# tohtsky/irspack

Measured on AMD Instinct MI355X. Metric: iALS user+item updates/sec at k=64, ML-20M-shape CSR, higher is better.
Workload: dtype f32; 1 GPU; ml20m-shape synthetic CSR 138493x26744 nnz=20004796, iALS k=64 fp32, solver=CHOLESKY; loss=IALSPP, balance=equal

## Files before the change

irspack_amd/csrc/ials.hip:

```cpp
#include <algorithm>
#include <chrono>
#include <cmath>
#include <cstdlib>
#include <atomic>
#include <cstring>
#include <map>
#include <memory>
#include <numeric>
#include <random>
#include <sstream>
#include <future>
#include <thread>

#include "common.hpp"
#include "comm.hpp"
#include "host_prep.hpp"

#include <hip/hip_ext.h>
#include "ials_kernels.hpp"
#include "ials_chol16.hpp"
#include "ials_wg_kernels.hpp"
#include "ials_wg16_kernels.hpp"
#include "ials_pp_kernels.hpp"
#include "ials_feature_kernels.hpp"
#include "ials_ridge_kernels.hpp"
#include "ials_short_kernels.hpp"
#include "ials_gk_kernels.hpp"
#include "ials_eig_kernels.hpp"
#include "ials_mf_kernels.hpp"

namespace irs {

std::string &last_error() {
  static thread_local std::string e;
  return e;
}

void require_device(int device) {
  int n = 0;
  hipError_t e = hipGetDeviceCount(&n);
  if (e != hipSuccess || n <= 0)
    throw std::runtime_error(
        "irspack_amd: no HIP device is visible; the gfx950 kernels cannot run "
        "(there is no CPU fallback).");
  if (device < 0 || device >= n)
    throw std::invalid_argument("irspack_amd: device index out of range.");
  IRS_HIP(hipSetDevice(device));
}

namespace ials {

static int padded_k(int64_t K) {
  if (K <= 16) return 16;
  if (K <= 32) return 32;
  if (K <= 64) return 64;
  return static_cast<int>(ceil_div(K, 64) * 64);
}

static int chunk_size() {
  static int v = [] {
    const char *e = std::getenv("IRSPACK_AMD_IALS_CHUNK");
    int c = e ? std::atoi(e) : 1024;
    if (c < 64) c = 64;
    return (c + 3) & ~3;
  }();
  return v;
}

static int max_chunks() { return 256; }

struct Side {
  int64_t n_rows = 0, n_other = 0, row_begin = 0, row_end = 0, nnz = 0;
  DeviceBuffer<int32_t> indptr, indices;
  DeviceBuffer<float> data, reg;
  DeviceBuffer<Task> tasks;
  DeviceBuffer<SplitRow> split;
  DeviceBuffer<FoldGroup> fold;
  int32_t n_fold = 0;
  DeviceBuffer<int32_t> rows_by_len;
  int32_t n_tasks = 0, n_split = 0, n_slots = 0, n_long = 0;
  int32_t n_short = 0, n_short16 = 0, n_short8 = 0;
  int64_t long_entries = 0;
  DeviceBuffer<MfLongRow> mf_lrows;
  DeviceBuffer<MfChunk> mf_chunks;
  int32_t mf_n_lrows = 0, mf_n_chunks = 0, mf_class[MF_CLASSES + 1] = {};
  bool unit = false;
  bool positive = false;
  float reg_min = 0.f;
  bool has_empty = false;
  bool entries_ready = false, indptr_ready = false;

  void alloc_entries(size_t ne, hipStream_t s) {
    indices.alloc(ne + 320);
    data.alloc(ne + 320);
    IRS_HIP(hipMemsetAsync(indices.ptr + ne, 0, 320 * sizeof(int32_t), s));
    IRS_HIP(hipMemsetAsync(data.ptr + ne, 0, 320 * sizeof(float), s));
    entries_ready = true;
  }
  void upload_entries(const HostCsr &m, hipStream_t s) {
    const size_t ne = static_cast<size_t>(m.indptr[m.rows]);
    alloc_entries(ne, s);
    if (ne) {
      IRS_HIP(hipMemcpyAsync(indices.ptr, m.idx(), ne * sizeof(int32_t), hipMemcpyHostToDevice, s));
      if (m.data.size() == ne) {
        IRS_HIP(hipMemcpyAsync(data.ptr, m.data.data(), ne * sizeof(float), hipMemcpyHostToDevice, s));
      } else {
        check_arg(m.flags_known && m.unit, "internal: a value array is missing.");
        IRS_HIP(hipMemsetD32Async(reinterpret_cast<hipDeviceptr_t>(data.ptr), 0x3f800000, ne, s));
      }
    }
    IRS_HIP(hipStreamSynchronize(s));
  }
  void upload_indptr(const HostCsr &m, hipStream_t s) {
    std::vector<int32_t> ip32(m.rows + 1);
    for (int64_t r = 0; r <= m.rows; r++) ip32[r] = static_cast<int32_t>(m.indptr[r]);
    indptr.upload(ip32, s);
    IRS_HIP(hipStreamSynchronize(s));
    indptr_ready = true;
  }

  void build(const HostCsr &m, int64_t rb, int64_t re, const irs_ials_model_config &cfg,
             hipStream_t s, const Side *share = nullptr) {
    n_rows = m.rows;
    n_other = m.cols;
    row_begin = rb;
    row_end = re;
    nnz = m.indptr[m.rows];
    if (share) {
      unit = share->unit;
// ... 79 lines not shown
      data.borrow(share->data);
    } else {
      if (!indptr_ready) indptr.upload(ip32, s);
      if (!entries_ready) upload_entries(m, s);
    }
    {
      std::vector<int32_t> order(re - rb);
      {
        int32_t max_len = 0;
        for (int64_t r = rb; r < re; r++) max_len = std::max(max_len, ip32[r + 1] - ip32[r]);
        std::vector<int32_t> start(static_cast<size_t>(max_len) + 2, 0);
        for (int64_t r = rb; r < re; r++) start[max_len - (ip32[r + 1] - ip32[r]) + 1]++;
        for (size_t i = 1; i < start.size(); i++) start[i] += start[i - 1];
        for (int64_t r = rb; r < re; r++)
          order[start[max_len - (ip32[r + 1] - ip32[r])]++] = static_cast<int32_t>(r);
      }
      rows_by_len.upload(order, s);
      if (cfg.K > 128 && cfg.K <= 256) {
        size_t i = 0;
        for (int c = 0; c < MF_CLASSES; c++) {
          mf_class[c] = static_cast<int32_t>(i);
          const int32_t lower = c + 1 < MF_CLASSES ? MF_CAPS[c + 1] : -1;
          while (i < order.size() && ip32[order[i] + 1] - ip32[order[i]] > lower) i++;
        }
        mf_class[MF_CLASSES] = static_cast<int32_t>(order.size());
        std::vector<MfLongRow> lr;
        std::vector<MfChunk> ch;
        for (int32_t k = 0; k < mf_class[1]; k++) {
          const int32_t r = order[k], b = ip32[r], e = ip32[r + 1], nz = e - b;
          const int32_t nch = (nz + MF_CHUNK - 1) / MF_CHUNK;
          const int32_t per = (((nz + nch - 1) / nch) + 15) & ~15;
          MfLongRow L{r, static_cast<int32_t>(ch.size()), 0, 0};
          for (int32_t c = b; c < e; c += per) {
            ch.push_back(MfChunk{k, c, std::min(c + per, e), 0});
            L.n_chunks++;
          }
          lr.push_back(L);
        }
        mf_n_lrows = static_cast<int32_t>(lr.size());
        mf_n_chunks = static_cast<int32_t>(ch.size());
        mf_lrows.upload(lr, s);
        mf_chunks.upload(ch, s);
        IRS_HIP(hipStreamSynchronize(s));
      }
      n_long = 0;
      while (n_long < static_cast<int32_t>(order.size()) &&
             ip32[order[n_long] + 1] - ip32[order[n_long]] > 2048)
        n_long++;
    }
    if (share) reg.borrow(share->reg);
    else reg.upload(regs, s);
    tasks.upload(tk, s);
    split.upload(sp, s);
    n_fold = static_cast<int32_t>(fg.size());
    fold.upload(fg, s);
    IRS_HIP(hipStreamSynchronize(s));
  }
};

struct Profiler {
  struct Rec {
    const char *name;
    hipEvent_t a, b;
  };
  bool enabled = false;
  bool dominant_only = false;
  const char *dominant_suffix = "_user";
  bool skip(const char *name) const {
    if (!enabled) return true;
    if (!dominant_only) return false;
    const size_t n = std::strlen(name), m = std::strlen(dominant_suffix);
    return std::strncmp(name, "ials_solve_", 11) != 0 || n < m || std::strcmp(name + n - m, dominant_suffix) != 0;
  }
  bool region_open = false;
  std::vector<Rec> recs;
  std::map<std::string, std::pair<double, int64_t>> totals;
  void begin(const char *name, hipStream_t s) {
    region_open = !skip(name);
    if (!region_open) return;
    Rec r{name, nullptr, nullptr};
    IRS_HIP(hipEventCreate(&r.a));
    IRS_HIP(hipEventCreate(&r.b));
    IRS_HIP(hipEventRecord(r.a, s));
    recs.push_back(r);
  }
  void end(hipStream_t s) {
    if (!region_open) return;
    region_open = false;
    IRS_HIP(hipEventRecord(recs.back().b, s));
  }
  template <class... Args, class F = void (*)(Args...)>
  void launch(const char *name, F kernel, dim3 grid, dim3 block, size_t lds, hipStream_t s, Args... args) {
    if (skip(name)) {
      hipLaunchKernelGGL(kernel, grid, block, lds, s, args...);
      return;
    }
    Rec r{name, nullptr, nullptr};
    IRS_HIP(hipEventCreate(&r.a));
    IRS_HIP(hipEventCreate(&r.b));
    if (dominant_only) {
      IRS_HIP(hipEventRecord(r.a, s));
      hipLaunchKernelGGL(kernel, grid, block, lds, s, args...);
      IRS_HIP(hipEventRecord(r.b, s));
    } else {
      hipExtLaunchKernelGGL(kernel, grid, block, static_cast<uint32_t>(lds), s, r.a, r.b, 0, args...);
    }
// ... 29 lines not shown
  int64_t K = 0, n_users = 0, n_items = 0;
  int KP = 0, T = 0;
  int device = 0;
  hipStream_t stream = nullptr;
  hipStream_t stream2 = nullptr;
  hipEvent_t ev_fork = nullptr, ev_join = nullptr;
  hipStream_t stream3 = nullptr;
  hipEvent_t ev_fork3 = nullptr, ev_join3 = nullptr;
  bool has_X = false;
  bool whole = true;
  irs_ials_shard shard{0, 0, 0, 0};
  DeviceBuffer<float> factor[2];
  Side side[2];
  DeviceBuffer<float> P_raw[2], P[2], P_acc[2], P_accL[2];
  DeviceBuffer<float> gram_partial, split_partial, row_loss;
  DeviceBuffer<double> loss_sum;
  DeviceBuffer<int32_t> err_flag;
  DeviceBuffer<float> prior[2];
  bool has_prior[2] = {false, false};
  int64_t n_feat[2] = {0, 0};
  DeviceBuffer<int32_t> f_indptr[2], f_indices[2], ft_indptr[2], ft_indices[2];
  DeviceBuffer<float> f_data[2], ft_data[2], f_W[2], f_rhs[2], f_part[2];
  int f_chunks[2] = {1, 1};
  int64_t w_rows[2] = {0, 0};
  DeviceBuffer<float> f_L[2], f_sol[2], f_gpart;
  bool ridge_ready[2] = {false, false};
  int64_t epoch = 0;
  DeviceBuffer<float> pp_pred;
  DeviceBuffer<int32_t> pp_llt_sink;
  DeviceBuffer<float> pp_pblk;
  DeviceBuffer<float> pp_px;
  DeviceBuffer<float> gk_sys, gk_delta;
  DeviceBuffer<float> eig_Qrows, eig_Qcols, eig_lam, eig_stats, eig_table, eig_xt, eig_xt2;
  DeviceBuffer<double> eig_Qd[2];
  bool eig_warm[2] = {false, false};
  int *eig_resident = nullptr;
  int eig_token = 0;
  float eig_stats_host[4] = {0, 0, 0, 0};
  bool opt_eig = true;
  DeviceBuffer<float> mf_vec, mf_xs, mf_rs, mf_partial, mf_r2;
  DeviceBuffer<int32_t> mf_done;
  bool opt_mf = true;
  bool gram_prefetched[2] = {false, false};
  std::vector<std::unique_ptr<Side>> chunk_side[2];
  int32_t eig_last = 0;
  bool gk() const { return KP > 256; }
  Profiler prof;
  bool opt_wave128 = true, opt_unit = true, opt_short = true, opt_wg16 = true;
  bool opt_short2 = true;
  bool opt_pp_direct = true;
  bool opt_pp_chain = true;
  bool opt_pp_fork = true;
  bool opt_bf16x3 = false;

  int64_t rows_of(int which) const { return which == 0 ? n_users : n_items; }
};

namespace {

#define IRS_DISPATCH_T(t, ...)                                                      \
  switch (t) {                                                                      \
    case 1: { constexpr int TT = 1; __VA_ARGS__; } break;                           \
    case 2: { constexpr int TT = 2; __VA_ARGS__; } break;                           \
    case 4: { constexpr int TT = 4; __VA_ARGS__; } break;                           \
    default:                                                                        \
      throw std::invalid_argument("irspack_amd: unsupported padded latent dimension."); \
  }
#define IRS_DISPATCH_T8(t, ...)                                                     \
  switch (t) {                                                                      \
    case 1: { constexpr int TT = 1; __VA_ARGS__; } break;                           \
    case 2: { constexpr int TT = 2; __VA_ARGS__; } break;                           \
    case 4: { constexpr int TT = 4; __VA_ARGS__; } break;                           \
    case 8: { constexpr int TT = 8; __VA_ARGS__; } break;                           \
    default:                                                                        \
      throw std::invalid_argument("irspack_amd: unsupported padded latent dimension."); \
  }
#define IRS_DISPATCH_TW(t, ...)                                                     \
  switch (t) {                                                                      \
    case 8: { constexpr int TT = 8; __VA_ARGS__; } break;                           \
    case 12: { constexpr int TT = 12; __VA_ARGS__; } break;                         \
    case 16: { constexpr int TT = 16; __VA_ARGS__; } break;                         \
    default:                                                                        \
      throw std::invalid_argument("irspack_amd: unsupported padded latent dimension."); \
  }
#define IRS_DISPATCH_ANY(t, ...)                                                    \
  switch (t) {                                                                      \
    case 1: { constexpr int TT = 1; __VA_ARGS__; } break;                           \
    case 2: { constexpr int TT = 2; __VA_ARGS__; } break;                           \
    case 4: { constexpr int TT = 4; __VA_ARGS__; } break;                           \
    case 8: { constexpr int TT = 8; __VA_ARGS__; } break;                           \
    case 12: { constexpr int TT = 12; __VA_ARGS__; } break;                         \
    case 16: { constexpr int TT = 16; __VA_ARGS__; } break;                         \
    default:                                                                        \
      throw std::invalid_argument("irspack_amd: unsupported padded latent dimension."); \
  }

void validate_config(const irs_ials_model_config &c) {
  check_arg(c.K >= 1, "K must be positive.");
  check_arg(c.K <= 32768, "irspack_amd: n_components above 32768 is not supported.");
  check_arg(c.loss_type == IRS_LOSS_ORIGINAL || c.loss_type == IRS_LOSS_IALSPP,
            "unknown loss_type.");
}

void read_switches(irs_ials_trainer *t);

void alloc_common(irs_ials_trainer *t) {
// ... 344 lines not shown
        PpParams ps = p;
        ps.rows = p.rows + n_long;
        ps.n_rows = n_rows - n_long;
        hipLaunchKernelGGL(kernel, dim3(ceil_div(ps.n_rows, 4)), dim3(256), lds, s2, ps);
      }
      if (fork) {
        IRS_HIP(hipEventRecord(t->ev_join, s2));
        IRS_HIP(hipStreamWaitEvent(t->stream, t->ev_join, 0));
      }
      t->prof.end(t->stream);
    }
  };
  const bool single = p.sub >= p.K;
  const bool chained = !single && TS == 4 && aligned && p.chain && p.sub == 64 && p.K > 64;
#define IRS_PP_LAUNCH(TSV, AL)                                                                        \
  do {                                                                                                \
    if (single)                                                                                       \
      launch(ialspp_long_kernel<TSV, AL, 1>, PpLongGeo<TSV>::LDS_FLOATS, ialspp_kernel<TSV, AL, 1>,   \
             PpGeo<TSV>::LDS_FLOATS);                                                                 \
    else                                                                                              \
      launch(ialspp_long_kernel<TSV, AL, 0>, PpLongGeo<TSV>::LDS_FLOATS, ialspp_kernel<TSV, AL, 0>,   \
             PpGeo<TSV>::LDS_FLOATS);                                                                 \
  } while (0)
  switch (TS * 2 + (aligned ? 1 : 0)) {
    case 2:
    case 3: IRS_PP_LAUNCH(1, true); break;
    case 4: IRS_PP_LAUNCH(2, false); break;
    case 5: IRS_PP_LAUNCH(2, true); break;
    case 8: IRS_PP_LAUNCH(4, false); break;
    default:
      if (chained)
        launch(ialspp_long_kernel<4, true, 2>, PpLongGeo<4>::LDS_FLOATS, ialspp_kernel<4, true, 2>,
               PpGeo<4>::LDS_FLOATS);
      else
        IRS_PP_LAUNCH(4, true);
      break;
  }
#undef IRS_PP_LAUNCH
  IRS_HIP(hipGetLastError());
}

void read_switches(irs_ials_trainer *t) {
  t->opt_wave128 = env_flag("IRSPACK_AMD_IALS_WAVE128", true);
  t->opt_unit = env_flag("IRSPACK_AMD_IALS_UNIT", true);
  t->opt_short = env_flag("IRSPACK_AMD_IALS_SHORT", true);
  t->opt_short2 = env_flag("IRSPACK_AMD_IALS_SHORT2", true);
  t->opt_pp_direct = env_flag("IRSPACK_AMD_IALSPP_DIRECT", true);
  t->opt_pp_chain = env_flag("IRSPACK_AMD_IALSPP_CHAIN", true);
  t->opt_pp_fork = env_flag("IRSPACK_AMD_IALSPP_FORK", true);
  t->opt_wg16 = env_flag("IRSPACK_AMD_IALS_WG16", true);
  t->opt_bf16x3 = env_flag("IRSPACK_AMD_IALS_BF16X3", true);
  t->opt_eig = env_flag("IRSPACK_AMD_IALS_EIG", true);
  t->opt_mf = env_flag("IRSPACK_AMD_IALS_MF", true);
}

void launch_eigen(irs_ials_trainer *t, int pidx, hipStream_t stream) {
  const int KP = t->KP;
  t->eig_Qrows.alloc(static_cast<size_t>(KP) * KP);
  t->eig_Qcols.alloc(static_cast<size_t>(KP) * KP);
  t->eig_lam.alloc(KP);
  t->eig_stats.alloc(4);
  t->eig_Qd[pidx].alloc(static_cast<size_t>(KP) * KP);
  if (!t->eig_resident) {
    IRS_HIP(hipHostMalloc(reinterpret_cast<void **>(&t->eig_resident), sizeof(int), hipHostMallocCoherent));
    *t->eig_resident = 0;
  }
  EigOut o{t->eig_Qrows.ptr, t->eig_Qcols.ptr, t->eig_lam.ptr, t->eig_stats.ptr, t->eig_Qd[pidx].ptr,
           t->eig_resident, ++t->eig_token};
  const int warm = t->eig_warm[pidx] ? 1 : 0;
  t->eig_warm[pidx] = true;
  const size_t lds = static_cast<size_t>(KP) * KP * sizeof(double);
  auto launch = [&](auto kernel) {
    IRS_HIP(hipFuncSetAttribute(reinterpret_cast<const void *>(kernel),
                                hipFuncAttributeMaxDynamicSharedMemorySize, static_cast<int>(lds)));
    t->prof.begin("eig_jacobi", stream);
    hipLaunchKernelGGL(kernel, dim3(1), dim3(1024), lds, stream,
                       static_cast<const float *>(t->P[pidx].ptr), static_cast<int>(t->K), o, warm);
    t->prof.end(stream);
  };
  if (KP == 128) launch(eig_jacobi_kernel<128>);
  else launch(eig_jacobi_kernel<64>);
  IRS_HIP(hipGetLastError());
}

bool eig_begin(irs_ials_trainer *t, Side &sd, int pidx, bool cg) {
  t->eig_last = 0;
  const int KP = t->KP;
  if (!t->opt_eig || (KP != 64 && KP != 128) || !sd.positive || sd.n_short <= 0) return false;
  if (static_cast<double>(sd.n_short) * KP * KP * KP < 3e11) return false;
  const double ratio = cg ? 64.0 : 8.0;
  if (static_cast<double>(sd.n_short) * KP < ratio * static_cast<double>(sd.n_other)) return false;
  if (!t->stream2) {
    IRS_HIP(hipStreamCreateWithFlags(&t->stream2, hipStreamNonBlocking));
    IRS_HIP(hipEventCreateWithFlags(&t->ev_fork, hipEventDisableTiming));
    IRS_HIP(hipEventCreateWithFlags(&t->ev_join, hipEventDisableTiming));
  }
  IRS_HIP(hipEventRecord(t->ev_fork, t->stream));
  IRS_HIP(hipStreamWaitEvent(t->stream2, t->ev_fork, 0));
  launch_eigen(t, pidx, t->stream2);
  const auto t0 = std::chrono::steady_clock::now();
  bool seen = false;
  int spins = 0;
  while (!(seen = __atomic_load_n(t->eig_resident, __ATOMIC_ACQUIRE) == t->eig_token) &&
         std::chrono::steady_clock::now() - t0 < std::chrono::milliseconds(200))
    if (++spins > 2000) std::this_thread::yield();
  if (!seen) {
// ... 334 lines not shown
    const int n_regular = sd.n_tasks - sd.n_short;
    int n_cu = 0;
    IRS_HIP(hipDeviceGetAttribute(&n_cu, hipDeviceAttributeMultiprocessorCount, t->device));
    t->prof.begin(pidx == 0 ? "ials_short_cg_user" : "ials_short_cg_item", short_stream);
    IRS_DISPATCH_T8(t->T, {
      constexpr int KPP = 16 * TT;
      const size_t lds = ShortGeo<KPP>::LDS_BYTES;
      auto launch = [&](auto kernel, int first, int count, int nr) {
        if (count <= 0) return;
        IRS_HIP(hipFuncSetAttribute(reinterpret_cast<const void *>(kernel),
                                    hipFuncAttributeMaxDynamicSharedMemorySize,
                                    static_cast<int>(lds)));
        const int grid = static_cast<int>(
            std::min<int64_t>(ceil_div(count, SHORT_WAVES * nr), 2 * std::max(n_cu, 1)));
        hipLaunchKernelGGL(kernel, dim3(grid), dim3(64 * SHORT_WAVES), lds, short_stream, p,
                           t->P[pidx].ptr, first, count);
      };
      if (t->opt_short2) {
        launch(ials_cg_short_kernel<KPP, 32, 1>, n_regular, sd.n_short - sd.n_short16, 1);
        launch(ials_cg_short_kernel<KPP, 16, 2>, sd.n_tasks - sd.n_short16, sd.n_short16, 2);
      } else {
        launch(ials_cg_short_kernel<KPP, 32, 1>, n_regular, sd.n_short - sd.n_short16, 1);
        launch(ials_cg_short_kernel<KPP, 16, 1>, sd.n_tasks - sd.n_short16, sd.n_short16, 1);
      }
    });
    t->prof.end(short_stream);
  };
  const bool eig_cand = prior == nullptr && !pp_direct && other == t->factor[1 - pidx].ptr &&
                        eig_begin(t, sd, pidx, cg);
  bool short_forked = false;
  if (eig_cand) {
    n_regular = sd.n_tasks - sd.n_short;
  } else if (short_cg_ok) {
    if (sd.n_short >= 65536) {
      if (!t->stream2) {
        IRS_HIP(hipStreamCreateWithFlags(&t->stream2, hipStreamNonBlocking));
        IRS_HIP(hipEventCreateWithFlags(&t->ev_fork, hipEventDisableTiming));
        IRS_HIP(hipEventCreateWithFlags(&t->ev_join, hipEventDisableTiming));
      }
      IRS_HIP(hipEventRecord(t->ev_fork, t->stream));
      IRS_HIP(hipStreamWaitEvent(t->stream2, t->ev_fork, 0));
      short_stream = t->stream2;
      short_forked = true;
    }
    launch_short_cg();
    short_stream = t->stream;
    n_regular = sd.n_tasks - sd.n_short;
  }
  auto fold_partials = [&](int partial_floats) {
    if (sd.n_fold <= 0) return;
    t->prof.launch("ials_fold_partials", fold_partials_kernel, dim3(sd.n_fold, ceil_div(partial_floats / 4, 256)),
                   dim3(256), 0, t->stream, t->split_partial.ptr, partial_floats, sd.fold.ptr);
  };
  auto launch_dense = [&](const Task *tasks_begin, int count, bool with_split) {
  const int n_regular = count;
  p.tasks = tasks_begin;
  p.n_tasks = count;
  if (!cg && (t->T >= 12 || (t->T == 8 && !t->opt_wave128)) && t->opt_wg16) {
    IRS_DISPATCH_TW(t->T, {
      using G = Geo<TT>;
      constexpr size_t lds = WgChol<TT>::LDS_FLOATS * sizeof(float);
      t->split_partial.alloc(static_cast<size_t>(std::max(sd.n_slots, 1)) * G::PARTIAL_FLOATS);
      p.partials = t->split_partial.ptr;
      auto launch = [&](auto kernel, int n_items, const char *name) {
        if (n_items <= 0) return;
        IRS_HIP(hipFuncSetAttribute(reinterpret_cast<const void *>(kernel),
                                    hipFuncAttributeMaxDynamicSharedMemorySize,
                                    static_cast<int>(lds)));
        t->prof.begin(name, t->stream);
        hipLaunchKernelGGL(kernel, dim3(n_items), dim3(256), lds, t->stream, p);
        t->prof.end(t->stream);
      };
      launch(ials_wg16_cholesky_kernel<TT, 0>, n_regular, kNames[0][0][pidx]);
      if (with_split) fold_partials(G::PARTIAL_FLOATS);
      if (with_split) launch(ials_wg16_cholesky_kernel<TT, 1>, sd.n_split, kNames[0][1][pidx]);
    });
  } else if (t->T == 8 && t->opt_wave128) {
    using G = Geo<8>;
    t->split_partial.alloc(static_cast<size_t>(std::max(sd.n_slots, 1)) * G::PARTIAL_FLOATS);
    p.partials = t->split_partial.ptr;
    if (n_regular > 0) {
      t->prof.begin(kNames[cg][0][pidx], t->stream);
      const bool x3_any = sd.unit && t->opt_unit && other == t->factor[1 - pidx].ptr && t->opt_bf16x3;
      const bool x3 = x3_any && (cg || sd.long_entries >= int64_t(320) * std::max(n_regular, 1));
      if (cg && x3)
        hipLaunchKernelGGL((ials_solve_kernel<8, 1, 0, true, true>), dim3(n_regular), dim3(64), 0, t->stream, p);
      else if (cg && unit)
        hipLaunchKernelGGL((ials_solve_kernel<8, 1, 0, true>), dim3(n_regular), dim3(64), 0, t->stream, p);
      else if (cg)
        hipLaunchKernelGGL((ials_solve_kernel<8, 1, 0>), dim3(n_regular), dim3(64), 0, t->stream, p);
      else if (x3)
        hipLaunchKernelGGL((ials_solve_kernel<8, 0, 0, true, true>), dim3(n_regular), dim3(64), 0, t->stream, p);
      else if (unit)
        hipLaunchKernelGGL((ials_solve_kernel<8, 0, 0, true>), dim3(n_regular), dim3(64), 0, t->stream, p);
      else
        hipLaunchKernelGGL((ials_solve_kernel<8, 0, 0>), dim3(n_regular), dim3(64), 0, t->stream, p);
      t->prof.end(t->stream);
    }
    if (with_split && sd.n_split > 0) {
      fold_partials(G::PARTIAL_FLOATS);
      t->prof.begin(kNames[cg][1][pidx], t->stream);
      if (cg && sd.unit && t->opt_unit && other == t->factor[1 - pidx].ptr && t->opt_bf16x3)
        hipLaunchKernelGGL((ials_solve_kernel<8, 1, 1, false, true>), dim3(sd.n_split), dim3(64), 0, t->stream, p);
      else if (cg)
        hipLaunchKernelGGL((ials_solve_kernel<8, 1, 1>), dim3(sd.n_split), dim3(64), 0, t->stream, p);
      else
        hipLaunchKernelGGL((ials_solve_kernel<8, 0, 1>), dim3(sd.n_split), dim3(64), 0, t->stream, p);
      t->prof.end(t->stream);
    }
  } else if (t->T <= 4) {
    IRS_DISPATCH_T(t->T, {
      using G = Geo<TT>;
      t->split_partial.alloc(static_cast<size_t>(std::max(sd.n_slots, 1)) * G::PARTIAL_FLOATS);
      p.partials = t->split_partial.ptr;
      if (n_regular > 0) {
        const dim3 grid(ceil_div(n_regular, SOLVE_WAVES)), block(64 * SOLVE_WAVES);
        const char *name = kNames[cg][0][pidx];
        if (pp_direct && unit && t->opt_bf16x3 && TT == 4)
          t->prof.launch(name, ials_solve_kernel<4, 0, 0, true, true, true>, grid, block, 0, t->stream, p);
        else if (pp_direct && unit)
          t->prof.launch(name, ials_solve_kernel<TT, 0, 0, true, false, true>, grid, block, 0, t->stream, p);
        else if (pp_direct)
          t->prof.launch(name, ials_solve_kernel<TT, 0, 0, false, false, true>, grid, block, 0, t->stream, p);
        else if (cg && unit && t->opt_bf16x3 && TT == 4)
          t->prof.launch(name, ials_solve_kernel<4, 1, 0, true, true>, grid, block, 0, t->stream, p);
        else if (cg && unit)
          t->prof.launch(name, ials_solve_kernel<TT, 1, 0, true>, grid, block, 0, t->stream, p);
        else if (cg)
          t->prof.launch(name, ials_solve_kernel<TT, 1, 0>, grid, block, 0, t->stream, p);
        else if (unit && t->opt_bf16x3 && TT == 4)
          t->prof.launch(name, ials_solve_kernel<4, 0, 0, true, true>, grid, block, 0, t->stream, p);
        else if (unit)
          t->prof.launch(name, ials_solve_kernel<TT, 0, 0, true>, grid, block, 0, t->stream, p);
        else
          t->prof.launch(name, ials_solve_kernel<TT, 0, 0>, grid, block, 0, t->stream, p);
      }
      if (with_split && sd.n_split > 0) {
        fold_partials(G::PARTIAL_FLOATS);
        const dim3 grid(ceil_div(sd.n_split, SOLVE_WAVES)), block(64 * SOLVE_WAVES);
        if (pp_direct)
          t->prof.launch(kNames[cg][1][pidx], ials_solve_kernel<TT, 0, 1, false, false, true>, grid, block, 0,
                         t->stream, p);
        else if (cg && unit && t->opt_bf16x3 && TT == 4)
          t->prof.launch(kNames[cg][1][pidx], ials_solve_kernel<4, 1, 1, false, true>, grid, block, 0, t->stream, p);
        else if (cg)
          t->prof.launch(kNames[cg][1][pidx], ials_solve_kernel<TT, 1, 1>, grid, block, 0, t->stream, p);
        else
          t->prof.launch(kNames[cg][1][pidx], ials_solve_kernel<TT, 0, 1>, grid, block, 0, t->stream, p);
      }
    });
  } else {
    IRS_DISPATCH_TW(t->T, {
      using G = Geo<TT>;
      constexpr size_t lds = WgGeo<TT>::LDS_FLOATS * sizeof(float);
      t->split_partial.alloc(static_cast<size_t>(std::max(sd.n_slots, 1)) * G::PARTIAL_FLOATS);
      p.partials = t->split_partial.ptr;
      auto launch = [&](auto kernel, int n_items, const char *name) {
        IRS_HIP(hipFuncSetAttribute(reinterpret_cast<const void *>(kernel),
                                    hipFuncAttributeMaxDynamicSharedMemorySize,
                                    static_cast<int>(lds)));
        t->prof.begin(name, t->stream);
        hipLaunchKernelGGL(kernel, dim3(n_items), dim3(256), lds, t->stream, p);
        t->prof.end(t->stream);
      };
      if (n_regular > 0) {
        if (cg)
          launch(ials_wg_solve_kernel<TT, 1, 0>, n_regular, kNames[1][0][pidx]);
        else
          launch(ials_wg_solve_kernel<TT, 0, 0>, n_regular, kNames[0][0][pidx]);
      }
      if (with_split && sd.n_split > 0) {
        fold_partials(G::PARTIAL_FLOATS);
        if (cg)
          launch(ials_wg_solve_kernel<TT, 1, 1>, sd.n_split, kNames[1][1][pidx]);
        else
          launch(ials_wg_solve_kernel<TT, 0, 1>, sd.n_split, kNames[0][1][pidx]);
      }
    });
  }
  IRS_HIP(hipGetLastError());
  };
  launch_dense(sd.tasks.ptr, n_regular, true);
  if (pp_direct) {
    for (uint64_t it = 1; it < sc->ialspp_iteration; it++) {
      pp_gramian_term();
      launch_dense(sd.tasks.ptr, n_regular, true);
    }
  }
  if (short_forked) {
    IRS_HIP(hipEventRecord(t->ev_join, t->stream2));
    IRS_HIP(hipStreamWaitEvent(t->stream, t->ev_join, 0));
  }
  if (eig_cand && !eig_finish(t, sd, other, target, pidx, cg, p.max_cg_steps, p.err_flag)) {
    p.tasks = sd.tasks.ptr;
    p.n_tasks = sd.n_tasks;
    if (short_cg_ok) launch_short_cg();
    else launch_dense(sd.tasks.ptr + n_regular, sd.n_short, false);
  }
}

void sync_and_check(irs_ials_trainer *t) {
  int32_t flag = 0;
  IRS_HIP(hipMemcpyAsync(&flag, t->err_flag.ptr, sizeof(flag), hipMemcpyDeviceToHost, t->stream));
  IRS_HIP(hipStreamSynchronize(t->stream));
  if (flag) {
    t->err_flag.zero(t->stream);
    IRS_HIP(hipStreamSynchronize(t->stream));
    if (flag & 1) throw std::runtime_error("Cholesky decomposition failed.");
    if (flag & 2) throw std::runtime_error("Cholesky solve failed.");
    if (flag & RIDGE_FLAG_CHOL)
      throw std::runtime_error("Feature ridge Cholesky decomposition failed.");
    if (flag & RIDGE_FLAG_SOLVE) throw std::runtime_error("Feature ridge solve failed.");
    if (flag & 8)
      throw std::runtime_error("The sharded step timed out waiting for a peer's stores.");
    throw std::runtime_error(
        "Conjugate-gradient solver encountered a singular system.");
  }
}

void require_X(irs_ials_trainer *t) {
  if (!t->has_X)
    throw std::runtime_error(
        "This IALSTrainer was restored from factors and holds no interaction matrix.");
}

void full_gramian(irs_ials_trainer *t, int side) {
  t->gram_prefetched[side] = false;
  const int other = 1 - side;
  const bool fused = t->T <= 4;
  launch_partial_gramian(t, other, 0, t->rows_of(other), side, fused);
  if (!fused) launch_finish_gramian(t, side);
}

}

extern "C" {

irs_status irs_ials_scores_device_(irs_ials_trainer *t, int64_t begin, int64_t end,
                                   float *device_out, void **stream_out, int32_t *device_index);
irs_status irs_ials_factors_device_(irs_ials_trainer *t, const float **user, const float **item,
                                    int32_t *KP, int64_t *n_users, int64_t *n_items,
                                    void **stream_out, int32_t *device_index);
irs_status irs_ials_scores_prefix_device_(irs_ials_trainer *t, int64_t begin, int64_t end,
                                          int64_t n_prefix, const float *item_rows,
                                          const float *user_rows, float *device_out);

const char *irs_last_error(void) { return irs::last_error().c_str(); }
int32_t irs_abi_version(void) { return IRS_ABI_VERSION; }
int32_t irs_device_count(void) {
  int n = 0;
  if (hipGetDeviceCount(&n) != hipSuccess) return 0;
  return n;
}

irs_status irs_ials_create(const irs_ials_model_config *config, int64_t n_users,
                           int64_t n_items, const int64_t *indptr, const int32_t *indices,
                           const float *data, int32_t device, const irs_ials_shard *shard,
                           irs_ials_trainer **out) {
  return guard([&] {
// ... 1084 lines not shown
```

irspack_amd/csrc/ials_kernels.hpp:

```cpp
#pragma once
#include <type_traits>
#include <hip/hip_runtime.h>

#include <cstdint>
#include <utility>

namespace irs {
namespace ials {

typedef float f32x4 __attribute__((ext_vector_type(4)));
typedef float f32x2 __attribute__((ext_vector_type(2)));

constexpr int SOLVE_WAVES = 1;

#ifndef SOLVE_MIN_WAVES_PER_SIMD
#define SOLVE_MIN_WAVES_PER_SIMD 2
#endif
#ifndef SOLVE_MIN_WAVES_PER_SIMD_K64
#define SOLVE_MIN_WAVES_PER_SIMD_K64 SOLVE_MIN_WAVES_PER_SIMD
#endif

struct Task {
  int32_t row;
  int32_t begin;
// ... 7 lines not shown
  int32_t n_slots;
  int32_t nnz;
  int32_t slot_stride;
};

constexpr int FOLD_GROUP = 16;
constexpr int FOLD_MIN = 32;
struct FoldGroup {
  int32_t first_slot;
  int32_t count;
};

__global__ __launch_bounds__(256) void fold_partials_kernel(float *__restrict__ partials, int partial_floats,
                                                            const FoldGroup *__restrict__ groups) {
  const FoldGroup g = groups[blockIdx.x];
  const int e = blockIdx.y * 256 + threadIdx.x;
  if (4 * e >= partial_floats) return;
  f32x4 *base = reinterpret_cast<f32x4 *>(partials + static_cast<size_t>(g.first_slot) * partial_floats) + e;
  const size_t step = static_cast<size_t>(partial_floats) / 4;
  f32x4 sum = base[0];
  int s = 1;
  for (; s + 4 <= g.count; s += 4) {
    const f32x4 a = base[s * step], b = base[(s + 1) * step], c = base[(s + 2) * step], d = base[(s + 3) * step];
    sum += a;
    sum += b;
    sum += c;
    sum += d;
  }
  for (; s < g.count; s++) sum += base[s * step];
  base[0] = sum;
}

struct SolveParams {
  const Task *tasks;
  int32_t n_tasks;
  const SplitRow *split_rows;
  int32_t n_split;
  const int32_t *indices;
  const float *data;
  const float *other;
  float *target;
  const float *reg;
  const float *P_acc;
  const float *P_accL;
  float *partials;
  int32_t *err_flag;
  float bias;
  int32_t K;
  int32_t max_cg_steps;
  int32_t warm_start;
  int32_t zero_row;
  const float *prior;
  const float *px = nullptr;
};

__device__ __forceinline__ int wave_in_block() {
  return __builtin_amdgcn_readfirstlane(static_cast<int>(threadIdx.x >> 6));
}

__device__ __forceinline__ float readlane_f(float x, int lane) {
  return __builtin_bit_cast(float, __builtin_amdgcn_readlane(__builtin_bit_cast(int, x), lane));
}

__device__ __forceinline__ float wave_sum(float v) {
#pragma unroll
  for (int off = 32; off >= 1; off >>= 1) v += __shfl_xor(v, off, 64);
  return v;
}

__device__ __forceinline__ float row16_sum(float x) {
  auto dpp = [](float v, auto ctrl) {
    return __builtin_bit_cast(float, __builtin_amdgcn_update_dpp(0, __builtin_bit_cast(int, v), decltype(ctrl)::value,
                                                                  0xf, 0xf, false));
  };
  x += dpp(x, std::integral_constant<int, 0xB1>{});
  x += dpp(x, std::integral_constant<int, 0x4E>{});
  x += dpp(x, std::integral_constant<int, 0x141>{});
  x += dpp(x, std::integral_constant<int, 0x140>{});
  return x;
}

template <int T> __device__ __forceinline__ void load_dims(const float *p, float (&v)[T]) {
  if constexpr (T == 4) {
    f32x4 t = *reinterpret_cast<const f32x4 *>(p);
    v[0] = t.x; v[1] = t.y; v[2] = t.z; v[3] = t.w;
  } else if constexpr (T == 2) {
    f32x2 t = *reinterpret_cast<const f32x2 *>(p);
    v[0] = t.x; v[1] = t.y;
  } else if constexpr (T == 1) {
    v[0] = *p;
  } else {
    static_assert(T % 4 == 0, "latent dims per lane must be 1, 2 or a multiple of 4");
#pragma unroll
    for (int q = 0; q < T / 4; q++) {
      f32x4 t = *reinterpret_cast<const f32x4 *>(p + 4 * q);
      v[4 * q] = t.x; v[4 * q + 1] = t.y; v[4 * q + 2] = t.z; v[4 * q + 3] = t.w;
    }
  }
}

template <int T>
__device__ __forceinline__ void add_prior(const SolveParams &p, int row, float (&bsum)[T]) {
  if (p.prior == nullptr) return;
  const int m = threadIdx.x & 15;
  const float reg = p.reg[row];
  float pr[T];
  load_dims<T>(p.prior + static_cast<size_t>(row) * (16 * T) + T * m, pr);
// ... 727 lines not shown
      break;
    }
    const float alpha = r2 / denom;
#pragma unroll
    for (int q = 0; q < 2; q++) {
      x[q] = fmaf(alpha, p[q], x[q]);
      r[q] = fmaf(-alpha, Ap[q], r[q]);
    }
    const float r2n = wave_sum(r[0] * r[0] + r[1] * r[1]);
    if (r2n <= 1e-20f) break;
    const float beta = r2n / r2;
#pragma unroll
    for (int q = 0; q < 2; q++) p[q] = fmaf(beta, p[q], r[q]);
  }
  if (singular) {
    if (lane == 0) atomicOr(err_flag, 4);
  }
#pragma unroll
  for (int q = 0; q < 2; q++) xrow[dim[q]] = act[q] ? x[q] : 0.f;
}

template <int T> struct Chol16Geo;
template <int T>
__device__ __forceinline__ void solve_row_cholesky16(f32x4 (&acc)[Geo<T>::NT], const float (&b4)[T],
                                                     float reg, float *sm, float *xrow, int K,
                                                     int32_t *err_flag);

#ifdef IRS_IALS_PHASES
__device__ unsigned long long ials_phase_clk[8 * 4096];
#define IPHASE(i) do { if ((threadIdx.x & 63) == 0) { const unsigned long long t_ = clock64(); atomicAdd(&ials_phase_clk[(i) * 4096 + (blockIdx.x & 4095)], t_ - ph_t); ph_t = t_; } } while (0)
#define IPHASE_BEGIN unsigned long long ph_t = clock64()
#else
#define IPHASE(i)
#define IPHASE_BEGIN
#endif

template <int T>
__device__ __forceinline__ void resid_finish_rhs(const SolveParams &p, int row, const float (&xr)[T], float (&bsum)[T]) {
  const int m = threadIdx.x & 15;
  const float reg = p.reg[row];
  float px[T];
  load_dims<T>(p.px + static_cast<size_t>(row) * (16 * T) + T * m, px);
#pragma unroll
  for (int i = 0; i < T; i++) bsum[i] -= fmaf(reg, xr[i], px[i]);
}
template <int T> __device__ __forceinline__ void resid_add_step(float *xrow, const float (&xr)[T]) {
  const int lane = threadIdx.x & 63;
  if (lane < 16) {
#pragma unroll
    for (int i = 0; i < T; i++) xrow[T * lane + i] += xr[i];
  }
}

template <int T, int SOLVER, int MODE, bool UNIT = false, bool BF16X3 = false, bool RESID = false>
__global__ __launch_bounds__(64 * SOLVE_WAVES, (T > 4 && (SOLVER == 1 || BF16X3)) ? 1 : (T <= 4 ? (RESID && MODE == 0 ? (UNIT ? 3 : 4) : (BF16X3 && MODE == 0 ? 3 : SOLVE_MIN_WAVES_PER_SIMD_K64)) : SOLVE_MIN_WAVES_PER_SIMD)) void ials_solve_kernel(SolveParams p) {
  static_assert(!BF16X3 || ((T == 4 || T == 8) && (MODE == 1 ? SOLVER == 1 : UNIT)),
                "bf16x3: unit confidences at 48 < K <= 64 and 64 < K <= 128");
  static_assert(!RESID || (SOLVER == 0 && T <= 4), "the gradient form: Cholesky at K <= 64");
  constexpr int WAVES = SOLVE_WAVES;
  using G = Geo<T>;
  constexpr bool LOWER = SOLVER == 0 || BF16X3;
  constexpr int RING = (T > 4 && SOLVER == 0) ? 4 : 8;
  constexpr int LDS_PER_WAVE = SOLVER == 0 ? Chol16Geo<T>::LDS_FLOATS
                                           : (T == 8 ? CholGeo<T>::SPILL_CG_FLOATS : G::CG_LDS_FLOATS);
  __shared__ __attribute__((aligned(16))) float lds[WAVES * LDS_PER_WAVE];
  const int wid = T <= 4 ? wave_in_block() : static_cast<int>(threadIdx.x >> 6);
  const int lane = threadIdx.x & 63;
  const int w = blockIdx.x * WAVES + wid;
  float *sm = lds + wid * LDS_PER_WAVE;

  f32x4 acc[G::NT];
  float bsum[T];
#pragma unroll
  for (int i = 0; i < T; i++) bsum[i] = 0.f;
  const f32x4 *Pacc = reinterpret_cast<const f32x4 *>(LOWER ? p.P_accL : p.P_acc);

  IPHASE_BEGIN;
  if constexpr (MODE == 0) {
    if (w >= p.n_tasks) return;
    const Task task = p.tasks[w];
    if (task.slot < 0) {
#pragma unroll
      for (int t = 0; t < G::NT; t++) acc[t] = Pacc[t * 64 + lane];
    } else {
#pragma unroll
      for (int t = 0; t < G::NT; t++) acc[t] = f32x4{0.f, 0.f, 0.f, 0.f};
    }
    float xr[T] = {};
    if constexpr (RESID) load_dims<T>(p.target + static_cast<size_t>(task.row) * G::KP + T * (lane & 15), xr);
    if constexpr (BF16X3)
      syrk_gather_bf16x3<T, RESID>(p.other, p.indices, task.begin, task.end, p.bias, acc, bsum,
                                   static_cast<unsigned>(p.zero_row), xr);
    else
      syrk_gather_impl<T, 1, 0, RING, UNIT, LOWER, RESID>(p.other, p.indices, p.data, task.begin, task.end, p.bias,
                                                          acc, bsum, static_cast<unsigned>(p.zero_row), xr);
    IPHASE(0);
    if (task.slot >= 0) {
      float *dst = p.partials + static_cast<size_t>(task.slot) * G::PARTIAL_FLOATS;
      f32x4 *d4 = reinterpret_cast<f32x4 *>(dst);
#pragma unroll
      for (int t = 0; t < G::NT; t++) d4[t * 64 + lane] = acc[t];
      if (lane < 16) {
#pragma unroll
        for (int i = 0; i < T; i++) dst[G::NT * 256 + T * lane + i] = bsum[i];
      }
      return;
    }
    add_prior<T>(p, task.row, bsum);
    if constexpr (RESID) resid_finish_rhs<T>(p, task.row, xr, bsum);
    const int nnz_cg = p.prior ? max(task.end - task.begin, 1) : task.end - task.begin;
    if constexpr (SOLVER == 0) {
      solve_row_cholesky16<T>(acc, bsum, p.reg[task.row], sm,
                              p.target + static_cast<size_t>(task.row) * G::KP, p.K, p.err_flag);
      if constexpr (RESID) resid_add_step<T>(p.target + static_cast<size_t>(task.row) * G::KP, xr);
    }
    else if constexpr (T == 8)
      solve_row_cg128<T, LOWER>(acc, bsum, p.reg[task.row], sm,
                         p.target + static_cast<size_t>(task.row) * G::KP, p.K, nnz_cg,
                         p.max_cg_steps, p.warm_start, p.err_flag);
    else
      solve_row<T, SOLVER, LOWER>(acc, bsum, p.reg[task.row], sm,
                           p.target + static_cast<size_t>(task.row) * G::KP, p.K, nnz_cg,
                           p.max_cg_steps, p.warm_start, p.err_flag);
  } else {
    if (w >= p.n_split) return;
    const SplitRow sr = p.split_rows[w];
#pragma unroll
    for (int t = 0; t < G::NT; t++) acc[t] = Pacc[t * 64 + lane];
    constexpr int U = T <= 4 ? 4 : 1;
    for (int s0 = 0; s0 < sr.n_slots; s0 += U) {
      f32x4 part[U][G::NT];
      float pb[U][T];
#pragma unroll
      for (int u = 0; u < U; u++) {
        const int s = min(s0 + u, sr.n_slots - 1);
        const float *src = p.partials + static_cast<size_t>(sr.first_slot + s * sr.slot_stride) * G::PARTIAL_FLOATS;
        const f32x4 *s4 = reinterpret_cast<const f32x4 *>(src);
#pragma unroll
        for (int t = 0; t < G::NT; t++) part[u][t] = s4[t * 64 + lane];
#pragma unroll
        for (int i = 0; i < T; i++) pb[u][i] = src[G::NT * 256 + T * (lane & 15) + i];
      }
#pragma unroll
      for (int u = 0; u < U; u++) {
        if (s0 + u < sr.n_slots) {
#pragma unroll
          for (int t = 0; t < G::NT; t++) acc[t] += part[u][t];
#pragma unroll
          for (int i = 0; i < T; i++) bsum[i] += pb[u][i];
        }
      }
    }
    add_prior<T>(p, sr.row, bsum);
    float xr[T] = {};
    if constexpr (RESID) {
      load_dims<T>(p.target + static_cast<size_t>(sr.row) * G::KP + T * (lane & 15), xr);
      resid_finish_rhs<T>(p, sr.row, xr, bsum);
    }
    if constexpr (SOLVER == 0) {
      solve_row_cholesky16<T>(acc, bsum, p.reg[sr.row], sm,
                              p.target + static_cast<size_t>(sr.row) * G::KP, p.K, p.err_flag);
      if constexpr (RESID) resid_add_step<T>(p.target + static_cast<size_t>(sr.row) * G::KP, xr);
    }
    else if constexpr (T == 8)
      solve_row_cg128<T, LOWER>(acc, bsum, p.reg[sr.row], sm,
                         p.target + static_cast<size_t>(sr.row) * G::KP, p.K, sr.nnz,
                         p.max_cg_steps, p.warm_start, p.err_flag);
    else
      solve_row<T, SOLVER, LOWER>(acc, bsum, p.reg[sr.row], sm,
                           p.target + static_cast<size_t>(sr.row) * G::KP, p.K, sr.nnz,
                           p.max_cg_steps, p.warm_start, p.err_flag);
  }
}

template <int T>
__global__ __launch_bounds__(256) void gramian_partial_kernel(const float *__restrict__ F,
                                                              int64_t row_begin,
                                                              int64_t row_end,
                                                              int64_t rows_per_wave,
                                                              float *__restrict__ partial) {
  using G = Geo<T>;
  const int lane = threadIdx.x & 63;
  const int g = lane >> 4, m = lane & 15;
  const int64_t w = static_cast<int64_t>(blockIdx.x) * 4 + wave_in_block();
  f32x4 acc[G::NT];
#pragma unroll
  for (int t = 0; t < G::NT; t++) acc[t] = f32x4{0.f, 0.f, 0.f, 0.f};
  const int64_t b = row_begin + w * rows_per_wave;
  const int64_t e = min(b + rows_per_wave, row_end);
  for (int64_t r = b; r < e; r += 4) {
    float v[T];
    if (r + g < e) {
      load_dims<T>(F + (r + g) * G::KP + T * m, v);
    } else {
#pragma unroll
      for (int i = 0; i < T; i++) v[i] = 0.f;
    }
    int t = 0;
#pragma unroll
    for (int i = 0; i < T; i++)
#pragma unroll
      for (int j = i; j < T; j++) {
        acc[t] = __builtin_amdgcn_mfma_f32_16x16x4f32(v[i], v[j], acc[t], 0, 0, 0);
        t++;
      }
  }
  __shared__ f32x4 fold[4 * G::NT * 64];
  const int wid = threadIdx.x >> 6;
#pragma unroll
  for (int t = 0; t < G::NT; t++) fold[(wid * G::NT + t) * 64 + lane] = acc[t];
  __syncthreads();
  f32x4 *dst = reinterpret_cast<f32x4 *>(partial) + static_cast<int64_t>(blockIdx.x) * (G::NT * 64);
  for (int e = threadIdx.x; e < G::NT * 64; e += 256) {
    f32x4 s = fold[e];
    s += fold[G::NT * 64 + e];
    s += fold[2 * G::NT * 64 + e];
    s += fold[3 * G::NT * 64 + e];
    dst[e] = s;
  }
}

constexpr int GRAM_CHAINS = 16;
template <int T, bool FINISH = false>
__global__ __launch_bounds__(64 * GRAM_CHAINS) void gramian_reduce_kernel(const float *__restrict__ partial,
// ... 206 lines not shown
```

Measured before the change: 96.72 million updates/s.

## Fuse split-row reduction into solve kernel via last-arriver ticket counters

Split rows' partial Gram/RHS contributions are written with cache-bypassing buffer stores. A per-split-row atomic ticket then lets the last finishing wave reduce all partials and solve the row inside the same kernel, so the separate split-solve launch is skipped when no fold groups exist. Host code builds a slot-to-split map and zeroes the ticket arrays, and resets them on error. It also raises the occupancy hint for the k=64 Cholesky solve kernel. The cost is atomics, fences and serialized tail work in the last-arriving wave.

```diff
diff --git a/irspack_amd/csrc/ials.hip b/irspack_amd/csrc/ials.hip
--- a/irspack_amd/csrc/ials.hip
+++ b/irspack_amd/csrc/ials.hip
@@ -75,6 +75,7 @@
   DeviceBuffer<float> data, reg;
   DeviceBuffer<Task> tasks;
   DeviceBuffer<SplitRow> split;
+  DeviceBuffer<int32_t> slot_split, tickets;
   DeviceBuffer<FoldGroup> fold;
   int32_t n_fold = 0;
   DeviceBuffer<int32_t> rows_by_len;
@@ -260,6 +261,16 @@
     else reg.upload(regs, s);
     tasks.upload(tk, s);
     split.upload(sp, s);
+    std::vector<int32_t> slot_sp(static_cast<size_t>(slots));
+    {
+      std::vector<int32_t> row_sp(static_cast<size_t>(re - rb), -1);
+      for (size_t i = 0; i < sp.size(); i++) row_sp[sp[i].row - rb] = static_cast<int32_t>(i);
+      for (const Task &a : tk)
+        if (a.slot >= 0) slot_sp[a.slot] = row_sp[a.row - rb];
+    }
+    slot_split.upload(slot_sp, s);
+    tickets.alloc(sp.size());
+    tickets.zero(s);
     n_fold = static_cast<int32_t>(fg.size());
     fold.upload(fg, s);
     IRS_HIP(hipStreamSynchronize(s));
@@ -395,6 +406,7 @@
   bool opt_pp_chain = true;
   bool opt_pp_fork = true;
   bool opt_bf16x3 = false;
+  bool opt_split_fused = true;
 
   int64_t rows_of(int which) const { return which == 0 ? n_users : n_items; }
 };
@@ -845,6 +857,7 @@
   t->opt_bf16x3 = env_flag("IRSPACK_AMD_IALS_BF16X3", true);
   t->opt_eig = env_flag("IRSPACK_AMD_IALS_EIG", true);
   t->opt_mf = env_flag("IRSPACK_AMD_IALS_MF", true);
+  t->opt_split_fused = env_flag("IRSPACK_AMD_IALS_SPLIT_FUSED", true);
 }
 
 void launch_eigen(irs_ials_trainer *t, int pidx, hipStream_t stream) {
@@ -1285,6 +1298,11 @@
     t->prof.launch("ials_fold_partials", fold_partials_kernel, dim3(sd.n_fold, ceil_div(partial_floats / 4, 256)),
                    dim3(256), 0, t->stream, t->split_partial.ptr, partial_floats, sd.fold.ptr);
   };
+  const bool split_fused = t->opt_split_fused && t->T <= 4 && sd.n_split > 0 && sd.n_fold == 0;
+  if (split_fused) {
+    p.slot_split = sd.slot_split.ptr;
+    p.tickets = sd.tickets.ptr;
+  }
   auto launch_dense = [&](const Task *tasks_begin, int count, bool with_split) {
   const int n_regular = count;
   p.tasks = tasks_begin;
@@ -1368,7 +1386,7 @@
         else
           t->prof.launch(name, ials_solve_kernel<TT, 0, 0>, grid, block, 0, t->stream, p);
       }
-      if (with_split && sd.n_split > 0) {
+      if (with_split && sd.n_split > 0 && !split_fused) {
         fold_partials(G::PARTIAL_FLOATS);
         const dim3 grid(ceil_div(sd.n_split, SOLVE_WAVES)), block(64 * SOLVE_WAVES);
         if (pp_direct)
@@ -1411,7 +1429,9 @@
       }
     });
   }
-  IRS_HIP(hipGetLastError());
+  const hipError_t launched = hipGetLastError();
+  if (launched != hipSuccess && split_fused) (void)hipMemsetAsync(sd.tickets.ptr, 0, sd.tickets.count * sizeof(int32_t), t->stream);
+  IRS_HIP(launched);
   };
   launch_dense(sd.tasks.ptr, n_regular, true);
   if (pp_direct) {
@@ -1438,6 +1458,10 @@
   IRS_HIP(hipStreamSynchronize(t->stream));
   if (flag) {
     t->err_flag.zero(t->stream);
+    for (int w = 0; w < 2; w++) {
+      t->side[w].tickets.zero(t->stream);
+      for (auto &cs : t->chunk_side[w]) cs->tickets.zero(t->stream);
+    }
     IRS_HIP(hipStreamSynchronize(t->stream));
     if (flag & 1) throw std::runtime_error("Cholesky decomposition failed.");
     if (flag & 2) throw std::runtime_error("Cholesky solve failed.");
diff --git a/irspack_amd/csrc/ials_kernels.hpp b/irspack_amd/csrc/ials_kernels.hpp
--- a/irspack_amd/csrc/ials_kernels.hpp
+++ b/irspack_amd/csrc/ials_kernels.hpp
@@ -83,7 +83,40 @@
   int32_t zero_row;
   const float *prior;
   const float *px = nullptr;
+  const int32_t *slot_split = nullptr;
+  int32_t *tickets = nullptr;
 };
+
+typedef unsigned int u32x4 __attribute__((ext_vector_type(4)));
+typedef unsigned int u32x2 __attribute__((ext_vector_type(2)));
+constexpr int AUX_SC1 = 16;
+__device__ __forceinline__ __amdgpu_buffer_rsrc_t partial_rsrc(const float *partial, int floats) {
+  return __builtin_amdgcn_make_buffer_rsrc(const_cast<float *>(partial), 0, floats * 4, 0x00020000);
+}
+template <int T> __device__ __forceinline__ void store_dims_sc1(__amdgpu_buffer_rsrc_t r, int byte_off, int base, const float (&v)[T]) {
+  if constexpr (T == 4)
+    __builtin_amdgcn_raw_buffer_store_b128(__builtin_bit_cast(u32x4, f32x4{v[0], v[1], v[2], v[3]}), r, byte_off, base, AUX_SC1);
+  else if constexpr (T == 2)
+    __builtin_amdgcn_raw_buffer_store_b64(__builtin_bit_cast(u32x2, f32x2{v[0], v[1]}), r, byte_off, base, AUX_SC1);
+  else {
+#pragma unroll
+    for (int i = 0; i < T; i++)
+      __builtin_amdgcn_raw_buffer_store_b32(__builtin_bit_cast(unsigned, v[i]), r, byte_off + 4 * i, base, AUX_SC1);
+  }
+}
+template <int T> __device__ __forceinline__ void load_dims_sc1(__amdgpu_buffer_rsrc_t r, int byte_off, int base, float (&v)[T]) {
+  if constexpr (T == 4) {
+    const f32x4 t = __builtin_bit_cast(f32x4, __builtin_amdgcn_raw_buffer_load_b128(r, byte_off, base, AUX_SC1));
+    v[0] = t.x; v[1] = t.y; v[2] = t.z; v[3] = t.w;
+  } else if constexpr (T == 2) {
+    const f32x2 t = __builtin_bit_cast(f32x2, __builtin_amdgcn_raw_buffer_load_b64(r, byte_off, base, AUX_SC1));
+    v[0] = t.x; v[1] = t.y;
+  } else {
+#pragma unroll
+    for (int i = 0; i < T; i++)
+      v[i] = __builtin_bit_cast(float, __builtin_amdgcn_raw_buffer_load_b32(r, byte_off + 4 * i, base, AUX_SC1));
+  }
+}
 
 __device__ __forceinline__ int wave_in_block() {
   return __builtin_amdgcn_readfirstlane(static_cast<int>(threadIdx.x >> 6));
@@ -917,8 +950,94 @@
   }
 }
 
+template <int T, int SOLVER, bool LOWER, bool RESID, int U, bool SC1>
+__device__ __forceinline__ void finish_split_row(const SolveParams &p, const SplitRow &sr, const f32x4 *Pacc,
+                                                 f32x4 (&acc)[Geo<T>::NT], float (&bsum)[T], float *sm) {
+  using G = Geo<T>;
+  int lane = threadIdx.x & 63;
+  if constexpr (SC1) asm volatile("" : "+v"(lane));
+#pragma unroll
+  for (int t = 0; t < G::NT; t++) acc[t] = Pacc[t * 64 + lane];
+  if constexpr (SC1 && U == 0) {
+    constexpr int H = (G::NT + 1) / 2;
+#pragma unroll 1
+    for (int s = 0; s < sr.n_slots; s++) {
+      const float *src = p.partials + static_cast<size_t>(sr.first_slot + s * sr.slot_stride) * G::PARTIAL_FLOATS;
+      const __amdgpu_buffer_rsrc_t rs = partial_rsrc(src, G::PARTIAL_FLOATS);
+      f32x4 part[H];
+      float pb[T];
+#pragma unroll
+      for (int t = 0; t < H; t++)
+        part[t] = __builtin_bit_cast(f32x4, __builtin_amdgcn_raw_buffer_load_b128(rs, lane * 16, t * 1024, AUX_SC1));
+      load_dims_sc1<T>(rs, T * (lane & 15) * 4, G::NT * 1024, pb);
+#pragma unroll
+      for (int t = 0; t < H; t++) acc[t] += part[t];
+#pragma unroll
+      for (int i = 0; i < T; i++) bsum[i] += pb[i];
+      asm volatile("" ::: "memory");
+#pragma unroll
+      for (int t = H; t < G::NT; t++)
+        part[t - H] = __builtin_bit_cast(f32x4, __builtin_amdgcn_raw_buffer_load_b128(rs, lane * 16, t * 1024, AUX_SC1));
+#pragma unroll
+      for (int t = H; t < G::NT; t++) acc[t] += part[t - H];
+    }
+  } else {
+#pragma unroll 1
+  for (int s0 = 0; s0 < sr.n_slots; s0 += U) {
+    f32x4 part[U][G::NT];
+    float pb[U][T];
+#pragma unroll
+    for (int u = 0; u < U; u++) {
+      const int s = min(s0 + u, sr.n_slots - 1);
+      const float *src = p.partials + static_cast<size_t>(sr.first_slot + s * sr.slot_stride) * G::PARTIAL_FLOATS;
+      if constexpr (SC1) {
+        const __amdgpu_buffer_rsrc_t rs = partial_rsrc(src, G::PARTIAL_FLOATS);
+#pragma unroll
+        for (int t = 0; t < G::NT; t++)
+          part[u][t] = __builtin_bit_cast(f32x4, __builtin_amdgcn_raw_buffer_load_b128(rs, lane * 16, t * 1024, AUX_SC1));
+        load_dims_sc1<T>(rs, T * (lane & 15) * 4, G::NT * 1024, pb[u]);
+      } else {
+        const f32x4 *s4 = reinterpret_cast<const f32x4 *>(src);
+#pragma unroll
+        for (int t = 0; t < G::NT; t++) part[u][t] = s4[t * 64 + lane];
+#pragma unroll
+        for (int i = 0; i < T; i++) pb[u][i] = src[G::NT * 256 + T * (lane & 15) + i];
+      }
+    }
+#pragma unroll
+    for (int u = 0; u < U; u++) {
+      if (s0 + u < sr.n_slots) {
+#pragma unroll
+        for (int t = 0; t < G::NT; t++) acc[t] += part[u][t];
+#pragma unroll
+        for (int i = 0; i < T; i++) bsum[i] += pb[u][i];
+      }
+    }
+  }
+  }
+  add_prior<T>(p, sr.row, bsum);
+  float xr[T] = {};
+  if constexpr (RESID) {
+    load_dims<T>(p.target + static_cast<size_t>(sr.row) * G::KP + T * (lane & 15), xr);
+    resid_finish_rhs<T>(p, sr.row, xr, bsum);
+  }
+  if constexpr (SOLVER == 0) {
+    solve_row_cholesky16<T>(acc, bsum, p.reg[sr.row], sm,
+                            p.target + static_cast<size_t>(sr.row) * G::KP, p.K, p.err_flag);
+    if constexpr (RESID) resid_add_step<T>(p.target + static_cast<size_t>(sr.row) * G::KP, xr);
+  }
+  else if constexpr (T == 8)
+    solve_row_cg128<T, LOWER>(acc, bsum, p.reg[sr.row], sm,
+                       p.target + static_cast<size_t>(sr.row) * G::KP, p.K, sr.nnz,
+                       p.max_cg_steps, p.warm_start, p.err_flag);
+  else
+    solve_row<T, SOLVER, LOWER>(acc, bsum, p.reg[sr.row], sm,
+                         p.target + static_cast<size_t>(sr.row) * G::KP, p.K, sr.nnz,
+                         p.max_cg_steps, p.warm_start, p.err_flag);
+}
+
 template <int T, int SOLVER, int MODE, bool UNIT = false, bool BF16X3 = false, bool RESID = false>
-__global__ __launch_bounds__(64 * SOLVE_WAVES, (T > 4 && (SOLVER == 1 || BF16X3)) ? 1 : (T <= 4 ? (RESID && MODE == 0 ? (UNIT ? 3 : 4) : (BF16X3 && MODE == 0 ? 3 : SOLVE_MIN_WAVES_PER_SIMD_K64)) : SOLVE_MIN_WAVES_PER_SIMD)) void ials_solve_kernel(SolveParams p) {
+__global__ __launch_bounds__(64 * SOLVE_WAVES, (T > 4 && (SOLVER == 1 || BF16X3)) ? 1 : (T <= 4 ? (RESID && MODE == 0 ? (UNIT ? 3 : 4) : (BF16X3 && MODE == 0 ? 3 : (SOLVER == 0 && MODE == 0 ? 4 : SOLVE_MIN_WAVES_PER_SIMD_K64))) : SOLVE_MIN_WAVES_PER_SIMD)) void ials_solve_kernel(SolveParams p) {
   static_assert(!BF16X3 || ((T == 4 || T == 8) && (MODE == 1 ? SOLVER == 1 : UNIT)),
                 "bf16x3: unit confidences at 48 < K <= 64 and 64 < K <= 128");
   static_assert(!RESID || (SOLVER == 0 && T <= 4), "the gradient form: Cholesky at K <= 64");
@@ -963,11 +1082,33 @@
     if (task.slot >= 0) {
       float *dst = p.partials + static_cast<size_t>(task.slot) * G::PARTIAL_FLOATS;
       f32x4 *d4 = reinterpret_cast<f32x4 *>(dst);
-#pragma unroll
-      for (int t = 0; t < G::NT; t++) d4[t * 64 + lane] = acc[t];
-      if (lane < 16) {
-#pragma unroll
-        for (int i = 0; i < T; i++) dst[G::NT * 256 + T * lane + i] = bsum[i];
+      if (T > 4 || p.tickets == nullptr) {
+#pragma unroll
+        for (int t = 0; t < G::NT; t++) d4[t * 64 + lane] = acc[t];
+        if (lane < 16) {
+#pragma unroll
+          for (int i = 0; i < T; i++) dst[G::NT * 256 + T * lane + i] = bsum[i];
+        }
+        return;
+      }
+      if constexpr (T <= 4) {
+        const int si = p.slot_split[task.slot];
+        const SplitRow sr = p.split_rows[si];
+        const __amdgpu_buffer_rsrc_t rs = partial_rsrc(dst, G::PARTIAL_FLOATS);
+#pragma unroll
+        for (int t = 0; t < G::NT; t++)
+          __builtin_amdgcn_raw_buffer_store_b128(__builtin_bit_cast(u32x4, acc[t]), rs, lane * 16, t * 1024, AUX_SC1);
+        if (lane < 16) store_dims_sc1<T>(rs, T * lane * 4, G::NT * 1024, bsum);
+        asm volatile("s_waitcnt vmcnt(0)" ::: "memory");
+        int ticket = 0;
+        if (lane == 0) ticket = __hip_atomic_fetch_add(p.tickets + si, 1, __ATOMIC_RELAXED, __HIP_MEMORY_SCOPE_AGENT);
+        ticket = __builtin_amdgcn_readfirstlane(ticket);
+        if (ticket != sr.n_slots - 1) return;
+        if (lane == 0) __hip_atomic_store(p.tickets + si, 0, __ATOMIC_RELAXED, __HIP_MEMORY_SCOPE_AGENT);
+        __builtin_amdgcn_fence(__ATOMIC_ACQUIRE, "agent");
+#pragma unroll
+        for (int i = 0; i < T; i++) bsum[i] = 0.f;
+        finish_split_row<T, SOLVER, LOWER, RESID, ((BF16X3 || T < 4) ? 2 : (SOLVER == 0 ? 0 : 1)), true>(p, sr, Pacc, acc, bsum, sm);
       }
       return;
     }
@@ -990,51 +1131,7 @@
   } else {
     if (w >= p.n_split) return;
     const SplitRow sr = p.split_rows[w];
-#pragma unroll
-    for (int t = 0; t < G::NT; t++) acc[t] = Pacc[t * 64 + lane];
-    constexpr int U = T <= 4 ? 4 : 1;
-    for (int s0 = 0; s0 < sr.n_slots; s0 += U) {
-      f32x4 part[U][G::NT];
-      float pb[U][T];
-#pragma unroll
-      for (int u = 0; u < U; u++) {
-        const int s = min(s0 + u, sr.n_slots - 1);
-        const float *src = p.partials + static_cast<size_t>(sr.first_slot + s * sr.slot_stride) * G::PARTIAL_FLOATS;
-        const f32x4 *s4 = reinterpret_cast<const f32x4 *>(src);
-#pragma unroll
-        for (int t = 0; t < G::NT; t++) part[u][t] = s4[t * 64 + lane];
-#pragma unroll
-        for (int i = 0; i < T; i++) pb[u][i] = src[G::NT * 256 + T * (lane & 15) + i];
-      }
-#pragma unroll
-      for (int u = 0; u < U; u++) {
-        if (s0 + u < sr.n_slots) {
-#pragma unroll
-          for (int t = 0; t < G::NT; t++) acc[t] += part[u][t];
-#pragma unroll
-          for (int i = 0; i < T; i++) bsum[i] += pb[u][i];
-        }
-      }
-    }
-    add_prior<T>(p, sr.row, bsum);
-    float xr[T] = {};
-    if constexpr (RESID) {
-      load_dims<T>(p.target + static_cast<size_t>(sr.row) * G::KP + T * (lane & 15), xr);
-      resid_finish_rhs<T>(p, sr.row, xr, bsum);
-    }
-    if constexpr (SOLVER == 0) {
-      solve_row_cholesky16<T>(acc, bsum, p.reg[sr.row], sm,
-                              p.target + static_cast<size_t>(sr.row) * G::KP, p.K, p.err_flag);
-      if constexpr (RESID) resid_add_step<T>(p.target + static_cast<size_t>(sr.row) * G::KP, xr);
-    }
-    else if constexpr (T == 8)
-      solve_row_cg128<T, LOWER>(acc, bsum, p.reg[sr.row], sm,
-                         p.target + static_cast<size_t>(sr.row) * G::KP, p.K, sr.nnz,
-                         p.max_cg_steps, p.warm_start, p.err_flag);
-    else
-      solve_row<T, SOLVER, LOWER>(acc, bsum, p.reg[sr.row], sm,
-                           p.target + static_cast<size_t>(sr.row) * G::KP, p.K, sr.nnz,
-                           p.max_cg_steps, p.warm_start, p.err_flag);
+    finish_split_row<T, SOLVER, LOWER, RESID, (T <= 4 ? 4 : 1), false>(p, sr, Pacc, acc, bsum, sm);
   }
 }
 
```

Result: no change. 96.14 million updates/s (-0.6%).
